# yinyunie/Pose2Room

Measured on AMD Instinct MI355X. Metric: P2RNet train-step samples/sec (T=1024,J=53,bs=32), higher is better.
Workload: dtype f32; 1 GPU; P2RNet full train step, bs=32/GPU, T=1024, J=53, seeds=512, proposals=128 (BASELINE configs[2]); input=P2RNet_dataloader over SyntheticPoseDataset, global_batch=32, frames=1024, parallelism=dp1

## Files before the change

pose2room_amd/p2rnet/modules/stgcn.py:

```python
import torch
import torch.nn as nn

from ..registers import MODULES
from .stgcn_layers import Graph, st_gcn_block
from .sub_modules import SingleConv


def _point_mlp(cin, width, cout):
    return nn.Sequential(SingleConv(cin, width, kernel_size=1, order='cbr', padding=0, ndim=1),
                         SingleConv(width, width, kernel_size=1, order='cbr', padding=0, ndim=1),
                         SingleConv(width, cout, kernel_size=1, order='c', padding=0, ndim=1))


@MODULES.register_module
class STGCN(nn.Module):
    def __init__(self, cfg, optim_spec=None):
        super().__init__()
        self.optim_spec = optim_spec

        self.graph = Graph(layout='virtualroom', strategy='spatial', max_hop=5)
        self.register_buffer('A', torch.tensor(self.graph.A, dtype=torch.float32, requires_grad=False))

        self.n_seeds = cfg.config['data']['num_seeds']
        self.origin_joint_id = cfg.dataset_config.origin_joint_id
        width, out_channels = 64, 256
        kernel_size = (3, self.A.size(0))
        self.knn = 20

        self.pos_embed = _point_mlp(3, 64, width)
        self.sk_feat = _point_mlp(3, 64, width)
        self.st_gcn_networks = nn.ModuleList(
            [st_gcn_block(width, 64, kernel_size, 1, residual=False)] +
            [st_gcn_block(64, 64, kernel_size, 1) for _ in range(5)])
        from ..gcn_op import GraphTables
        tables = GraphTables(self.graph.A)
        for i, blk in enumerate(self.st_gcn_networks):
            blk.gcn.tables = tables
            blk.chain_input = i > 0
        self.conv_joint = nn.Conv1d(cfg.dataset_config.joint_num * 64, out_channels, kernel_size=1)
        self.edge_importance = nn.ParameterList(
            [nn.Parameter(torch.ones(self.A.size())) for _ in self.st_gcn_networks])

        n_frames = cfg.config['data']['num_frames']
        if self.n_seeds >= n_frames:
            self.seed_inds = torch.round(torch.linspace(0, n_frames - 1, self.n_seeds)).long()
        else:
            self.seed_sampling = cfg.config['data']['seed_sampling']

    def _select_seeds(self, hip):
        n_batch, n_frames, _ = hip.shape
        device = hip.device
        if self.n_seeds >= n_frames:
            return self.seed_inds.repeat(n_batch, 1).to(device)
        if self.seed_sampling == 'random':
            inds = torch.argsort(torch.rand(size=(n_batch, n_frames)), dim=1)[:, :self.n_seeds]
            return torch.sort(inds, dim=1)[0].to(device)
        if self.seed_sampling == 'uniform':
            step = torch.norm(torch.diff(hip, dim=1), dim=2)
            cum = torch.cumsum(torch.cat([torch.zeros(size=(n_batch, 1), device=device), step], dim=1).double(),
                               dim=1).float()
            stride = cum[:, -1] / (self.n_seeds - 1)
            target = stride.unsqueeze(-1) * torch.arange(self.n_seeds, dtype=torch.float, device=device)
            if cum.is_cuda and cum.dtype == torch.float32 and n_frames <= 40000:
                from .. import seed_op
                return seed_op.nearest_prefix(cum, target)
            return torch.argmin(torch.abs(cum.unsqueeze(-1) - target.unsqueeze(1)), dim=1)
        raise NotImplementedError

    @staticmethod
    def _mlp(seq, x, inner, add_ct=None):
        from .. import bn_op, tconv_op, embed_op
        if embed_op.supported(seq, x, inner, add_ct):
            return embed_op.embed_mlp(seq, x, inner, add_ct)
        s0, s1, s2 = seq
        fused = (x.is_cuda and len(seq) == 3 and hasattr(s0, 'batchnorm') and hasattr(s1, 'batchnorm')
                 and not hasattr(s2, 'batchnorm') and tconv_op.supported_embed3(x, s0.conv)
                 and x.shape[2] % inner == 0 and inner <= 64)
        if fused:
            z0s = None
            if s0.batchnorm.training:
                z, z0s = tconv_op.embed3(x, s0.conv, want_stats=True)
            else:
                z = tconv_op.embed3(x, s0.conv)
            z = z.view(x.shape[0], 64, x.shape[2] // inner, inner)
            fused = tconv_op.supported_pointwise(z, s0.batchnorm, s1.conv) and \
                tconv_op.supported_pointwise(z, s1.batchnorm, s2.conv)
            if fused:
                if s1.batchnorm.training:
                    z, zs = tconv_op.bn_relu_tconv(z, s0.batchnorm, s1.conv, stats=z0s, want_stats=True)
                    z = tconv_op.bn_relu_tconv(z, s1.batchnorm, s2.conv, stats=zs, add_ct=add_ct)
                else:
                    z = tconv_op.bn_relu_tconv(z, s0.batchnorm, s1.conv)
                    z = tconv_op.bn_relu_tconv(z, s1.batchnorm, s2.conv, add_ct=add_ct)
                return z.view(x.shape[0], 64, x.shape[2])
        for stage in seq:
            if x.is_cuda and hasattr(stage, 'batchnorm') and hasattr(stage, 'ReLU') and \
                    bn_op.supported(x, stage.batchnorm):
                x = bn_op.fused_bn_act(stage.conv(x), stage.batchnorm, None, relu=True)
            else:
                x = stage(x)
        if add_ct is not None:
            x = (x.view(x.shape[0], x.shape[1], -1, inner) + add_ct.unsqueeze(-1)).view(x.shape)
        return x

    def embed(self, input_joints):
        n_batch, n_frames, n_joints, _ = input_joints.shape
        device = input_joints.device
        hip = input_joints[:, :, self.origin_joint_id]
        win = torch.arange(n_frames, device=device).unsqueeze(-1) + \
            torch.arange(-self.knn // 2, self.knn // 2, device=device).unsqueeze(0)
        win = win.clamp_(0, n_frames - 1)
        offs = hip[:, win] - hip.unsqueeze(2)
        pe = self._mlp(self.pos_embed, offs.reshape(n_batch, n_frames * self.knn, 3).transpose(1, 2).contiguous(), self.knn)
        from .. import seed_op
        pe = pe.view(n_batch, -1, n_frames, self.knn)
        fused = seed_op.short_rows_supported(pe)
        pe = seed_op.mean_last(pe) if fused else pe.mean(dim=3)
        rel = input_joints - input_joints[:, :, self.origin_joint_id:self.origin_joint_id + 1]
        sk = self._mlp(self.sk_feat, rel.reshape(n_batch, n_frames * n_joints, 3).transpose(1, 2).contiguous(), n_joints,
                       add_ct=pe)
        return sk.view(n_batch, -1, n_frames, n_joints)

    def forward(self, input_joints, end_points=None):
        end_points = {} if end_points is None else end_points
        n_batch, n_frames, n_joints, n_dim = input_joints.size()
        seed_inds = self._select_seeds(input_joints[:, :, self.origin_joint_id])

        x = self.embed(input_joints)
        blocks = self.st_gcn_networks
        tables = blocks[0].gcn.tables
        if tables is not None and tables.gen2 and all(b.chainable(x, self.A) for b in blocks):
            from ..gcn_op import prepare_chain
            for gcn, prep in zip(blocks, prepare_chain(blocks, self.A, self.edge_importance, tables, frames=x.shape[2])):
                x, _ = gcn(x, prep.Aeff, prepared=prep)
        else:
            for gcn, importance in zip(blocks, self.edge_importance):
                x, _ = gcn(x, self.A * importance)

        seed_skeleton = torch.gather(
            input_joints, 1, seed_inds[:, :, None, None].expand(n_batch, self.n_seeds, n_joints, n_dim))
        if self.n_seeds < n_frames:
            from .. import seed_op
            if seed_op.seed_rows_supported(x, seed_inds):
                rows = seed_op.seed_rows(x, seed_inds)
            else:
                rows = x.permute(0, 2, 1, 3)[torch.arange(n_batch, device=x.device)[:, None], seed_inds]
            seed_features = torch.nn.functional.linear(
                rows.reshape(n_batch, self.n_seeds, -1),
                self.conv_joint.weight.squeeze(-1), self.conv_joint.bias)
        else:
            x = x.transpose(2, 3).reshape(n_batch, -1, n_frames)
            seed_features = self.conv_joint(x).transpose(1, 2)
            seed_features = torch.gather(
                seed_features, 1, seed_inds.unsqueeze(-1).expand(n_batch, self.n_seeds, seed_features.size(-1)))
        end_points['seed_inds'] = seed_inds
        end_points['seed_skeleton'] = seed_skeleton[..., :3]
        end_points['seed_features'] = seed_features
        return end_points
```

pose2room_amd/p2rnet/modules/stgcn_layers.py:

```python
from collections import deque

import numpy as np
import torch
import torch.nn as nn

_VIRTUALROOM_BONES = [
    (0, 1), (1, 3), (3, 5), (5, 19), (0, 2), (2, 4), (4, 6), (6, 20), (0, 7), (7, 8), (8, 9),
    (9, 10), (10, 21), (10, 22), (8, 11), (11, 13), (13, 15), (15, 17), (8, 12), (12, 14),
    (14, 16), (16, 18), (17, 23), (23, 24), (24, 25), (17, 26), (26, 27), (27, 28), (17, 29),
    (29, 30), (30, 31), (17, 32), (32, 33), (33, 34), (17, 35), (35, 36), (36, 37), (18, 38),
    (38, 39), (39, 40), (18, 41), (41, 42), (42, 43), (18, 44), (44, 45), (45, 46), (18, 47),
    (47, 48), (48, 49), (18, 50), (50, 51), (51, 52)]

_LAYOUTS = {'virtualroom': dict(num_node=53, bones=_VIRTUALROOM_BONES, center=0)}


def hop_distance(num_node, edges, max_hop):
    nbr = [[] for _ in range(num_node)]
    for i, j in edges:
        if i != j:
            nbr[i].append(j)
            nbr[j].append(i)
    hop = np.full((num_node, num_node), np.inf)
    for s in range(num_node):
        hop[s, s] = 0
        dq = deque([s])
        while dq:
            u = dq.popleft()
            if hop[s, u] >= max_hop:
                continue
            for v in nbr[u]:
                if np.isinf(hop[s, v]):
                    hop[s, v] = hop[s, u] + 1
                    dq.append(v)
    return hop


class Graph:

    def __init__(self, layout='virtualroom', strategy='spatial', max_hop=5, dilation=1):
        if layout not in _LAYOUTS:
            raise ValueError("Do Not Exist This Layout.")
        spec = _LAYOUTS[layout]
        self.max_hop, self.dilation = max_hop, dilation
        self.num_node, self.center = spec['num_node'], spec['center']
        self.edge = [(i, i) for i in range(self.num_node)] + list(spec['bones'])
        self.hop_dis = hop_distance(self.num_node, self.edge, max_hop)
        self.A = self._adjacency(strategy)

    def _adjacency(self, strategy):
        V = self.num_node
        hops = list(range(0, self.max_hop + 1, self.dilation))
        reach = np.zeros((V, V))
        for h in hops:
            reach[self.hop_dis == h] = 1
        col = reach.sum(0)
        inv = np.zeros(V)
        inv[col > 0] = col[col > 0] ** (-1)
        norm = reach * inv[None, :]
        if strategy == 'uniform':
            return norm[None]
        if strategy == 'distance':
            return np.stack([np.where(self.hop_dis == h, norm, 0.0) for h in hops])
        if strategy == 'spatial':
            dc = self.hop_dis[:, self.center]
            same = dc[:, None] == dc[None, :]
            closer = dc[:, None] > dc[None, :]
            planes = []
            for h in hops:
                at_h = self.hop_dis == h
                root = np.where(at_h & same, norm, 0.0)
                close = np.where(at_h & closer, norm, 0.0)
                further = np.where(at_h & ~same & ~closer, norm, 0.0)
                if h == 0:
                    planes.append(root)
                else:
                    planes.append(root + close)
                    planes.append(further)
            return np.stack(planes)
        raise ValueError("Do Not Exist This Strategy")


class ConvTemporalGraphical(nn.Module):

    def __init__(self, in_channels, out_channels, kernel_size, t_kernel_size=1, t_stride=1,
                 t_padding=0, t_dilation=1, bias=True):
        super().__init__()
        self.kernel_size = kernel_size
        self.out_channels = out_channels
        self.tables = None
        self.fused = True
        self.conv = nn.Conv2d(in_channels, out_channels * kernel_size, kernel_size=(t_kernel_size, 1),
                              padding=(t_padding, 0), stride=(t_stride, 1), dilation=(t_dilation, 1),
                              bias=bias)

    def forward(self, x, A, want_stats=False, with_residual=False, bn_link=None, prepared=None, lazy_res=False):
        assert A.size(0) == self.kernel_size
        if self.tables is not None and self.fused:
            from .. import gcn_op
            if gcn_op.supported(x, self.conv.weight, A):
                return gcn_op.graph_conv(x, self.conv.weight, self.conv.bias, A, self.tables, want_stats,
                                         with_residual, bn_link, prepared, lazy_res), A
        assert not want_stats and not with_residual and prepared is None
        y = self.conv(x)
        n, kc, t, v = y.size()
        y = y.view(n, self.kernel_size, kc // self.kernel_size, t, v)
        z = torch.einsum('nkctv,kvw->nctw', (y, A))
        return z.contiguous(), A


def _zero(x):
    return 0


def _iden(x):
    return x


class st_gcn_block(nn.Module):

    def __init__(self, in_channels, out_channels, kernel_size, stride=1, dropout=0, residual=True):
        super().__init__()
        assert len(kernel_size) == 2 and kernel_size[0] % 2 == 1
        padding = ((kernel_size[0] - 1) // 2, 0)
        self.gcn = ConvTemporalGraphical(in_channels, out_channels, kernel_size[1])
        self.tcn = nn.Sequential(
            nn.BatchNorm2d(out_channels),
            nn.ReLU(inplace=True),
            nn.Conv2d(out_channels, out_channels, (kernel_size[0], 1), (stride, 1), padding),
            nn.BatchNorm2d(out_channels),
            nn.Dropout(dropout, inplace=True),
        )
        if not residual:
            self.residual = _zero
        elif in_channels == out_channels and stride == 1:
            self.residual = _iden
        else:
            self.residual = nn.Sequential(
                nn.Conv2d(in_channels, out_channels, kernel_size=1, stride=(stride, 1)),
                nn.BatchNorm2d(out_channels))
        self.relu = nn.ReLU(inplace=True)

    fused_bn = True
    fused_tconv = True
    lazy_residual_grad = True
    chain_input = False

    def chainable(self, x, A):
        if not (self.fused_bn and x.is_cuda and self.tcn[4].p == 0):
            return False
        from .. import bn_op, gcn_op, tconv_op
        return (self.training and self.fused_tconv and self.gcn.tables is not None and self.gcn.fused
                and gcn_op.supported(x, self.gcn.conv.weight, A) and bn_op.supported(x, self.tcn[0])
                and tconv_op.supported(x, self.tcn[0], self.tcn[2]))

    def forward(self, x, A, prepared=None):
        res = self.residual(x)
        if self.fused_bn and x.is_cuda and self.tcn[4].p == 0:
            from .. import bn_op, gcn_op, tconv_op
            chain = self.chainable(x, A)
            assert chain or prepared is None
            lazy = False
            if chain:
                if self.residual is _iden and x.requires_grad:
                    in_link = getattr(x, '_p2r_bn_link', None) if self.chain_input else None
                    lazy = self.lazy_residual_grad and self.tcn[3].training
                    (z, zstats, res), A = self.gcn(x, A, want_stats=True, with_residual=True, bn_link=in_link,
                                                   prepared=prepared, lazy_res=lazy)
                else:
                    (z, zstats), A = self.gcn(x, A, want_stats=True, prepared=prepared)
                wp = (prepared.tcn_wp_f, prepared.tcn_wp_b) if prepared is not None and z.shape[3] == 53 else None
                u, ustats = tconv_op.bn_relu_tconv(z, self.tcn[0], self.tcn[2], stats=zstats, want_stats=True, wp=wp)
                res_t = res if torch.is_tensor(res) else None
                return bn_op.fused_bn_act(u, self.tcn[3], res_t, relu=True, stats=ustats, link=bn_op.BNLink(),
                                          lazy_res=lazy), A
            x, A = self.gcn(x, A)
            if bn_op.supported(x, self.tcn[0]):
                if self.fused_tconv and tconv_op.supported(x, self.tcn[0], self.tcn[2]):
                    u = tconv_op.bn_relu_tconv(x, self.tcn[0], self.tcn[2])
                else:
                    h = bn_op.fused_bn_act(x, self.tcn[0], None, relu=True)
                    u = self.tcn[2](h)
                res_t = res if torch.is_tensor(res) else None
                return bn_op.fused_bn_act(u, self.tcn[3], res_t, relu=True), A
        else:
            x, A = self.gcn(x, A)
        x = self.tcn(x) + res
        return self.relu(x), A
```

pose2room_amd/p2rnet/seed_op.py:

```python
import torch
from torch.autograd import Function

from .. import _lib


def _rowsum(x, V, scale):
    out = torch.empty(x.shape[:-1], dtype=torch.float32, device=x.device)
    _lib.launch("p2r_rowsum_short", x.device, x.numel() // V, V, scale, x, out)
    return out


def short_rows_supported(x):
    return x.is_cuda and x.dtype == torch.float32 and 1 <= x.shape[-1] <= 64


class _SeedRows(Function):

    @staticmethod
    def forward(ctx, x, seed_inds):
        x = x.contiguous()
        inds = seed_inds.long().contiguous()
        B, C, T, J = x.shape
        S = inds.shape[1]
        out = torch.empty((B, S, C * J), dtype=torch.float32, device=x.device)
        _lib.launch("p2r_gather_frames", x.device, B, C, T, J, S, x, inds, out)
        ctx.save_for_backward(inds)
        ctx.dims = (B, C, T, J, S)
        return out

    @staticmethod
    def backward(ctx, dout):
        (inds,) = ctx.saved_tensors
        B, C, T, J, S = ctx.dims
        dout = dout.contiguous()
        dx = torch.empty((B, C, T, J), dtype=torch.float32, device=dout.device)
        _lib.launch("p2r_gather_frames_grad", dout.device, B, C, T, J, S, dout, inds, dx)
        return dx, None


def seed_rows_supported(x, seed_inds):
    return (x.is_cuda and x.dtype == torch.float32 and x.dim() == 4 and seed_inds.is_cuda and seed_inds.dim() == 2
            and seed_inds.dtype in (torch.int64, torch.int32) and seed_inds.shape[0] == x.shape[0])


def seed_rows(x, seed_inds):
    return _SeedRows.apply(x, seed_inds)


class _MeanLast(Function):

    @staticmethod
    def forward(ctx, x):
        x = x.contiguous()
        ctx.shape = x.shape
        return _rowsum(x, x.shape[-1], 1.0 / x.shape[-1])

    @staticmethod
    def backward(ctx, g):
        return (g * (1.0 / ctx.shape[-1])).unsqueeze(-1).expand(ctx.shape)


def mean_last(x):
    return _MeanLast.apply(x)


class _AddBroadcastLast(Function):

    @staticmethod
    def forward(ctx, a, b):
        ctx.V = a.shape[-1]
        return a + b.unsqueeze(-1)

    @staticmethod
    def backward(ctx, g):
        db = None
        if ctx.needs_input_grad[1]:
            gc = g.contiguous()
            db = _rowsum(gc, ctx.V, 1.0)
        return (g if ctx.needs_input_grad[0] else None), db


def add_broadcast_last(a, b):
    return _AddBroadcastLast.apply(a, b)


def nearest_prefix(cum, target):
    cum, target = cum.contiguous(), target.contiguous()
    B, T = cum.shape
    S = target.shape[1]
    out = torch.empty((B, S), dtype=torch.int64, device=cum.device)
    _lib.launch("p2r_nearest_prefix", cum.device, B, T, S, cum, target, out)
    return out
```

Before: 796.3 samples/s.

## Fuse last ST-GCN block BN+ReLU with seed-frame gather, skip full activation

In training, the final ST-GCN block's output BN+residual+ReLU is now fused with the seed-row gather. It computes activations only at the selected seed frames instead of writing the full B×C×T×J tensor and gathering from it afterwards. The backward pass builds a per-frame linked list of seed indices so duplicate seeds are handled, then runs a BN-statistics reduce kernel and an apply kernel that produce du and dres directly. This saves one full-size write and read in forward, but backward still streams over the full activation and adds an index-building kernel, a uint8 mask, and a second shared library.

```diff
diff --git a/include/p2r_seed_seam.h b/include/p2r_seed_seam.h
--- /dev/null
+++ b/include/p2r_seed_seam.h
@@ -0,0 +1,23 @@
+#ifndef P2R_SEED_SEAM_H
+#define P2R_SEED_SEAM_H
+
+#include "p2r_hip.h"
+
+#ifdef __cplusplus
+extern "C" {
+#endif
+
+int p2r_seam_apply_gather(int b, int c, int t, int j, int s, const float *u, const float *res, const float *scale,
+                          const float *shift, const long long *inds, float *rows, unsigned char *mask, void *stream);
+int p2r_seam_index(int b, int t, int s, const long long *inds, int *head, int *next, void *stream);
+int p2r_seam_bwd_reduce(int b, int c, int t, int j, int s, const float *drows, const unsigned char *mask,
+                        const float *u, const float *mean, const float *invstd, const int *head, const int *next,
+                        float *partial, void *stream);
+int p2r_seam_bwd_apply(int b, int c, int t, int j, int s, const float *drows, const unsigned char *mask,
+                       const float *u, const float *mean, const float *invstd, const float *kscale, const float *m1,
+                       const float *m2, const int *head, const int *next, float *du, float *dres, void *stream);
+
+#ifdef __cplusplus
+}
+#endif
+#endif
diff --git a/pose2room_amd/csrc/seed_seam.hip b/pose2room_amd/csrc/seed_seam.hip
--- /dev/null
+++ b/pose2room_amd/csrc/seed_seam.hip
@@ -0,0 +1,271 @@
+#include "p2r_common.h"
+
+#include "../../include/p2r_seed_seam.h"
+
+namespace {
+
+constexpr int SS_THREADS = 256;
+constexpr int SS_MAX_T = 8192;
+
+typedef float f4v __attribute__((ext_vector_type(4)));
+__device__ __forceinline__ float4 ld_stream(const float *p) {
+  const f4v t = __builtin_nontemporal_load(reinterpret_cast<const f4v *>(p));
+  return make_float4(t.x, t.y, t.z, t.w);
+}
+__device__ __forceinline__ void st_stream(float *p, const float4 &v) {
+  __builtin_nontemporal_store(f4v{v.x, v.y, v.z, v.w}, reinterpret_cast<f4v *>(p));
+}
+
+__global__ __launch_bounds__(SS_THREADS) void seam_index_kernel(int T, int S, const long long *__restrict__ inds,
+                                                               int *__restrict__ head, int *__restrict__ next) {
+  __shared__ long long tile[SS_THREADS];
+  const int b = blockIdx.y, tid = threadIdx.x;
+  const int nT = (T + SS_THREADS - 1) / SS_THREADS;
+  const long long *ib = inds + (size_t)b * S;
+  const bool frames = (int)blockIdx.x < nT;
+  const int id = (frames ? (int)blockIdx.x : (int)blockIdx.x - nT) * SS_THREADS + tid;
+  long long want = -1;
+  int from = 0;
+  if (frames) {
+    if (id < T) want = id;
+  } else if (id < S) {
+    const long long t = ib[id];
+    if (t >= 0 && t < T) want = t;
+    from = id + 1;
+  }
+  int found = -1;
+  for (int s0 = frames ? 0 : ((int)blockIdx.x - nT) * SS_THREADS; s0 < S; s0 += SS_THREADS) {
+    __syncthreads();
+    tile[tid] = s0 + tid < S ? ib[s0 + tid] : -1;
+    __syncthreads();
+    if (want >= 0 && found < 0) {
+      const int n = min(SS_THREADS, S - s0);
+      for (int k = max(0, from - s0); k < n; ++k)
+        if (tile[k] == want) { found = s0 + k; break; }
+    }
+  }
+  if (frames) {
+    if (id < T) head[(size_t)b * T + id] = found;
+  } else if (id < S) {
+    next[(size_t)b * S + id] = found;
+  }
+}
+
+__global__ __launch_bounds__(SS_THREADS) void seam_apply_gather_kernel(int C, int T, int J, int S,
+                                                                      const float *__restrict__ u,
+                                                                      const float *__restrict__ res,
+                                                                      const float *__restrict__ scale,
+                                                                      const float *__restrict__ shift,
+                                                                      const long long *__restrict__ inds,
+                                                                      float *__restrict__ rows,
+                                                                      unsigned char *__restrict__ mask) {
+  const int b = blockIdx.x / S;
+  const long long t = inds[blockIdx.x];
+  const int n = C * J;
+  float *o = rows + (size_t)blockIdx.x * n;
+  unsigned char *m = mask + (size_t)blockIdx.x * n;
+  if (t < 0 || t >= T) {
+    for (int e = threadIdx.x; e < n; e += SS_THREADS) { o[e] = 0.f; m[e] = 0; }
+    return;
+  }
+  const size_t fb = ((size_t)b * C * T + t) * J;
+  for (int e = threadIdx.x; e < n; e += SS_THREADS) {
+    const int c = e / J, j = e - c * J;
+    const size_t at = fb + (size_t)c * T * J + j;
+    float v = fmaf(u[at], scale[c], shift[c]);
+    if (res) v += res[at];
+    v = fmaxf(v, 0.f);
+    o[e] = v;
+    m[e] = v > 0.f;
+  }
+}
+
+__device__ __forceinline__ float seam_gated(const float *__restrict__ rows_c, const unsigned char *__restrict__ mask_c,
+                                            const int *__restrict__ next_b, int S, int h, int n, int j) {
+  const size_t at = (size_t)h * n + j;
+  float g = rows_c[at];
+  const unsigned char m = mask_c[at];
+  for (int nx = next_b[h]; nx >= 0 && nx < S; nx = next_b[nx]) g += rows_c[(size_t)nx * n + j];
+  return m ? g : 0.f;
+}
+
+__device__ __forceinline__ float ss_wave_sum(float v) {
+#pragma unroll
+  for (int off = 32; off >= 1; off >>= 1) v += __shfl_xor(v, off, 64);
+  return v;
+}
+
+__global__ __launch_bounds__(SS_THREADS) void seam_bwd_reduce_kernel(int C, int T, int J, int S,
+                                                                    const float *__restrict__ drows,
+                                                                    const unsigned char *__restrict__ mask,
+                                                                    const float *__restrict__ u,
+                                                                    const float *__restrict__ mean,
+                                                                    const float *__restrict__ invstd,
+                                                                    const int *__restrict__ head,
+                                                                    const int *__restrict__ next,
+                                                                    float2 *__restrict__ partial) {
+  extern __shared__ int s_head[];
+  __shared__ float sa[SS_THREADS / 64], sb[SS_THREADS / 64];
+  const int row = blockIdx.x, b = row / C, c = row - b * C, tid = threadIdx.x;
+  for (int t = tid; t < T; t += SS_THREADS) s_head[t] = head[(size_t)b * T + t];
+  __syncthreads();
+  const float mu = mean[c], is = invstd[c];
+  const int L = T * J, n = C * J;
+  const size_t base = (size_t)row * L;
+  const float *rows_c = drows + (size_t)b * S * n + (size_t)c * J;
+  const unsigned char *mask_c = mask + (size_t)b * S * n + (size_t)c * J;
+  const int *next_b = next + (size_t)b * S;
+  auto term = [&](int e, int t, int j, float &g, float &gx) {
+    const int h = s_head[t];
+    g = 0.f; gx = 0.f;
+    if (h >= 0 && h < S) {
+      g = seam_gated(rows_c, mask_c, next_b, S, h, n, j);
+      gx = g * ((u[base + e] - mu) * is);
+    }
+  };
+  float s = 0.f, q = 0.f;
+  const int L4 = (base % 4 == 0) ? (L >> 2) : 0;
+  for (int i = tid; i < L4; i += SS_THREADS) {
+    const int e = 4 * i;
+    int t = e / J, j = e - t * J;
+    float g[4], gx[4];
+#pragma unroll
+    for (int k = 0; k < 4; ++k) {
+      term(e + k, t, j, g[k], gx[k]);
+      if (++j == J) { j = 0; ++t; }
+    }
+    s += (g[0] + g[1]) + (g[2] + g[3]);
+    q += (gx[0] + gx[1]) + (gx[2] + gx[3]);
+  }
+  for (int e = (L4 << 2) + tid; e < L; e += SS_THREADS) {
+    const int t = e / J;
+    float g, gx;
+    term(e, t, e - t * J, g, gx);
+    s += g; q += gx;
+  }
+  s = ss_wave_sum(s);
+  q = ss_wave_sum(q);
+  if ((tid & 63) == 0) { sa[tid >> 6] = s; sb[tid >> 6] = q; }
+  __syncthreads();
+  if (tid == 0) {
+    s = 0.f; q = 0.f;
+#pragma unroll
+    for (int i = 0; i < SS_THREADS / 64; ++i) { s += sa[i]; q += sb[i]; }
+    partial[row] = make_float2(s, q);
+  }
+}
+
+__global__ __launch_bounds__(SS_THREADS) void seam_bwd_apply_kernel(int C, int T, int J, int S, int chunks,
+                                                                   const float *__restrict__ drows,
+                                                                   const unsigned char *__restrict__ mask,
+                                                                   const float *__restrict__ u,
+                                                                   const float *__restrict__ mean,
+                                                                   const float *__restrict__ invstd,
+                                                                   const float *__restrict__ kscale,
+                                                                   const float *__restrict__ m1,
+                                                                   const float *__restrict__ m2,
+                                                                   const int *__restrict__ head,
+                                                                   const int *__restrict__ next,
+                                                                   float *__restrict__ du, float *__restrict__ dres) {
+  const int rowi = blockIdx.x / chunks, chunk = blockIdx.x % chunks;
+  const int b = rowi / C, c = rowi - b * C;
+  const float mu = mean[c], is = invstd[c], kk = kscale[c], a1 = m1[c], a2 = m2[c];
+  const int L = T * J, n = C * J;
+  const size_t base = (size_t)rowi * L;
+  const int per = (((L + chunks - 1) / chunks) + 3) & ~3;
+  const int lo = chunk * per, hi = min(L, lo + per);
+  const float *rows_c = drows + (size_t)b * S * n + (size_t)c * J;
+  const unsigned char *mask_c = mask + (size_t)b * S * n + (size_t)c * J;
+  const int *next_b = next + (size_t)b * S, *head_b = head + (size_t)b * T;
+  auto one = [&](int t, int j, float xv, float &dxo, float &dro) {
+    const int h = head_b[t];
+    const float g = (h >= 0 && h < S) ? seam_gated(rows_c, mask_c, next_b, S, h, n, j) : 0.f;
+    const float xh = (xv - mu) * is;
+    dxo = kk * (g - a1 - xh * a2);
+    dro = g;
+  };
+  const bool vec = (((uintptr_t)(u + base) | (uintptr_t)(du + base) | (dres ? (uintptr_t)(dres + base) : 0)) % 16 == 0);
+  int tail = lo;
+  if (vec) {
+    tail = lo + ((hi - lo) & ~3);
+    for (int e = lo + threadIdx.x * 4; e + 3 < hi; e += SS_THREADS * 4) {
+      const float4 x4 = ld_stream(u + base + e);
+      const float xs[4] = {x4.x, x4.y, x4.z, x4.w};
+      float o[4], r[4];
+      int t = e / J, j = e - t * J;
+#pragma unroll
+      for (int k = 0; k < 4; ++k) {
+        one(t, j, xs[k], o[k], r[k]);
+        if (++j == J) { j = 0; ++t; }
+      }
+      st_stream(du + base + e, make_float4(o[0], o[1], o[2], o[3]));
+      if (dres) st_stream(dres + base + e, make_float4(r[0], r[1], r[2], r[3]));
+    }
+  }
+  for (int e = tail + threadIdx.x; e < hi; e += SS_THREADS) {
+    const int t = e / J;
+    float o, r;
+    one(t, e - t * J, u[base + e], o, r);
+    du[base + e] = o;
+    if (dres) dres[base + e] = r;
+  }
+}
+
+static int seam_chunks(int rows, int L) {
+  int chunks = 1;
+  while ((long long)rows * chunks < 2048 && (L / (chunks * 2)) >= 4096) chunks *= 2;
+  return chunks;
+}
+
+static bool seam_dims_ok(int b, int c, int t, int j, int s) {
+  return b >= 0 && c > 0 && t > 0 && j > 0 && s > 0 && (long long)t * j <= 0x7fffffffLL && (long long)c * j <= 0x7fffffffLL &&
+         (long long)b * c <= 0x7fffffffLL && (long long)b * s <= 0x7fffffffLL;
+}
+
+}
+
+extern "C" int p2r_seam_index(int b, int t, int s, const long long *inds, int *head, int *next, void *stream) {
+  if (b < 0 || t <= 0 || s <= 0 || b > 65535) return P2R_EINVAL;
+  if (b == 0) return P2R_OK;
+  const unsigned nx = (unsigned)((t + SS_THREADS - 1) / SS_THREADS + (s + SS_THREADS - 1) / SS_THREADS);
+  hipLaunchKernelGGL(seam_index_kernel, dim3(nx, (unsigned)b), dim3(SS_THREADS), 0, p2r_stream(stream), t, s, inds, head, next);
+  P2R_LAUNCH_CHECK();
+  return P2R_OK;
+}
+
+extern "C" int p2r_seam_apply_gather(int b, int c, int t, int j, int s, const float *u, const float *res, const float *scale,
+                                     const float *shift, const long long *inds, float *rows, unsigned char *mask,
+                                     void *stream) {
+  if (!seam_dims_ok(b, c, t, j, s)) return P2R_EINVAL;
+  if (b == 0) return P2R_OK;
+  hipLaunchKernelGGL(seam_apply_gather_kernel, dim3((unsigned)(b * s)), dim3(SS_THREADS), 0, p2r_stream(stream), c, t, j, s, u,
+                     res, scale, shift, inds, rows, mask);
+  P2R_LAUNCH_CHECK();
+  return P2R_OK;
+}
+
+extern "C" int p2r_seam_bwd_reduce(int b, int c, int t, int j, int s, const float *drows, const unsigned char *mask,
+                                   const float *u, const float *mean, const float *invstd, const int *head, const int *next,
+                                   float *partial, void *stream) {
+  if (!seam_dims_ok(b, c, t, j, s) || t > SS_MAX_T) return P2R_EINVAL;
+  if (b == 0) return P2R_OK;
+  hipLaunchKernelGGL(seam_bwd_reduce_kernel, dim3((unsigned)(b * c)), dim3(SS_THREADS), (size_t)t * sizeof(int),
+                     p2r_stream(stream), c, t, j, s, drows, mask, u, mean, invstd, head, next,
+                     reinterpret_cast<float2 *>(partial));
+  P2R_LAUNCH_CHECK();
+  return P2R_OK;
+}
+
+extern "C" int p2r_seam_bwd_apply(int b, int c, int t, int j, int s, const float *drows, const unsigned char *mask,
+                                  const float *u, const float *mean, const float *invstd, const float *kscale,
+                                  const float *m1, const float *m2, const int *head, const int *next, float *du, float *dres,
+                                  void *stream) {
+  if (!seam_dims_ok(b, c, t, j, s)) return P2R_EINVAL;
+  if (b == 0) return P2R_OK;
+  const int rows = b * c, chunks = seam_chunks(rows, t * j);
+  if ((long long)rows * chunks > 0x7fffffffLL) return P2R_EINVAL;
+  hipLaunchKernelGGL(seam_bwd_apply_kernel, dim3((unsigned)(rows * chunks)), dim3(SS_THREADS), 0, p2r_stream(stream), c, t, j, s,
+                     chunks, drows, mask, u, mean, invstd, kscale, m1, m2, head, next, du, dres);
+  P2R_LAUNCH_CHECK();
+  return P2R_OK;
+}
diff --git a/pose2room_amd/p2rnet/modules/stgcn.py b/pose2room_amd/p2rnet/modules/stgcn.py
--- a/pose2room_amd/p2rnet/modules/stgcn.py
+++ b/pose2room_amd/p2rnet/modules/stgcn.py
@@ -129,10 +129,14 @@
         x = self.embed(input_joints)
         blocks = self.st_gcn_networks
         tables = blocks[0].gcn.tables
+        rows = None
         if tables is not None and tables.gen2 and all(b.chainable(x, self.A) for b in blocks):
             from ..gcn_op import prepare_chain
+            seam = self.n_seeds < n_frames and blocks[-1].seam_supported(x, self.A, seed_inds)
             for gcn, prep in zip(blocks, prepare_chain(blocks, self.A, self.edge_importance, tables, frames=x.shape[2])):
-                x, _ = gcn(x, prep.Aeff, prepared=prep)
+                x, _ = gcn(x, prep.Aeff, prepared=prep, seed_inds=seed_inds if seam and gcn is blocks[-1] else None)
+            if seam:
+                rows, x = x, None
         else:
             for gcn, importance in zip(blocks, self.edge_importance):
                 x, _ = gcn(x, self.A * importance)
@@ -141,7 +145,9 @@
             input_joints, 1, seed_inds[:, :, None, None].expand(n_batch, self.n_seeds, n_joints, n_dim))
         if self.n_seeds < n_frames:
             from .. import seed_op
-            if seed_op.seed_rows_supported(x, seed_inds):
+            if rows is not None:
+                pass
+            elif seed_op.seed_rows_supported(x, seed_inds):
                 rows = seed_op.seed_rows(x, seed_inds)
             else:
                 rows = x.permute(0, 2, 1, 3)[torch.arange(n_batch, device=x.device)[:, None], seed_inds]
diff --git a/pose2room_amd/p2rnet/modules/stgcn_layers.py b/pose2room_amd/p2rnet/modules/stgcn_layers.py
--- a/pose2room_amd/p2rnet/modules/stgcn_layers.py
+++ b/pose2room_amd/p2rnet/modules/stgcn_layers.py
@@ -154,17 +154,25 @@
                 and gcn_op.supported(x, self.gcn.conv.weight, A) and bn_op.supported(x, self.tcn[0])
                 and tconv_op.supported(x, self.tcn[0], self.tcn[2]))
 
-    def forward(self, x, A, prepared=None):
+    def seam_supported(self, x, A, seed_inds):
+        if not (self.fused_bn and x.is_cuda and self.tcn[4].p == 0 and self.residual is _iden):
+            return False
+        from .. import seed_op
+        from torch.nn.modules import module as _m
+        hooked = bool(self._forward_hooks) or bool(_m._global_forward_hooks)
+        return not hooked and self.chainable(x, A) and seed_op.seam_supported(x, self.tcn[3], seed_inds)
+
+    def forward(self, x, A, prepared=None, seed_inds=None):
         res = self.residual(x)
         if self.fused_bn and x.is_cuda and self.tcn[4].p == 0:
-            from .. import bn_op, gcn_op, tconv_op
+            from .. import bn_op, gcn_op, seed_op, tconv_op
             chain = self.chainable(x, A)
-            assert chain or prepared is None
+            assert chain or (prepared is None and seed_inds is None)
             lazy = False
             if chain:
                 if self.residual is _iden and x.requires_grad:
                     in_link = getattr(x, '_p2r_bn_link', None) if self.chain_input else None
-                    lazy = self.lazy_residual_grad and self.tcn[3].training
+                    lazy = self.lazy_residual_grad and self.tcn[3].training and seed_inds is None
                     (z, zstats, res), A = self.gcn(x, A, want_stats=True, with_residual=True, bn_link=in_link,
                                                    prepared=prepared, lazy_res=lazy)
                 else:
@@ -172,6 +180,8 @@
                 wp = (prepared.tcn_wp_f, prepared.tcn_wp_b) if prepared is not None and z.shape[3] == 53 else None
                 u, ustats = tconv_op.bn_relu_tconv(z, self.tcn[0], self.tcn[2], stats=zstats, want_stats=True, wp=wp)
                 res_t = res if torch.is_tensor(res) else None
+                if seed_inds is not None:
+                    return seed_op.bn_act_seed_rows(u, self.tcn[3], res_t, seed_inds, stats=ustats), A
                 return bn_op.fused_bn_act(u, self.tcn[3], res_t, relu=True, stats=ustats, link=bn_op.BNLink(),
                                           lazy_res=lazy), A
             x, A = self.gcn(x, A)
diff --git a/pose2room_amd/p2rnet/seed_op.py b/pose2room_amd/p2rnet/seed_op.py
--- a/pose2room_amd/p2rnet/seed_op.py
+++ b/pose2room_amd/p2rnet/seed_op.py
@@ -1,3 +1,6 @@
+import ctypes
+import os
+
 import torch
 from torch.autograd import Function
 
@@ -47,6 +50,97 @@
     return _SeedRows.apply(x, seed_inds)
 
 
+SEAM_HEADER_PATH = os.path.join(os.path.dirname(_lib.HEADER_PATH), "p2r_seed_seam.h")
+SEAM_LIB_PATH = os.path.join(os.path.dirname(os.path.abspath(_lib.__file__)), "libp2r_seed_seam.so")
+_seam_lib = None
+_seam_protos = None
+
+
+def seam_lib():
+    global _seam_lib, _seam_protos
+    if _seam_lib is None:
+        if not os.path.exists(SEAM_LIB_PATH):
+            raise _lib.P2RLibraryError(f"{SEAM_LIB_PATH} is missing: build it with `make -C pose2room_amd/csrc` "
+                                       "(pose2room_amd has no CPU fallback)")
+        l = ctypes.CDLL(SEAM_LIB_PATH)
+        _seam_protos = _lib.prototypes(SEAM_HEADER_PATH)
+        for name, proto in _seam_protos.items():
+            fn = getattr(l, name)
+            fn.restype, fn.argtypes = proto.restype, proto.argtypes
+        _seam_lib = l
+    return _seam_lib
+
+
+def seam_launch(name, device, *args):
+    l = seam_lib()
+    proto = _seam_protos[name]
+    if len(args) != len(proto.pointer):
+        raise TypeError(f"{name}: {len(args)} arguments for {len(proto.pointer)} parameters in front of the stream: {proto.text}")
+    vals = [(a.data_ptr() if a is not None else None) if p else int(a) for a, p in zip(args, proto.pointer)]
+    if device.index is None or device.index == torch.cuda.current_device():
+        _lib.check(getattr(l, name)(*vals, _lib.current_stream(device)), name)
+    else:
+        with torch.cuda.device(device):
+            _lib.check(getattr(l, name)(*vals, _lib.current_stream(device)), name)
+
+
+FUSE_SEAM = True
+SEAM_MAX_FRAMES = 8192
+
+
+class _SeamBNAct(Function):
+
+    @staticmethod
+    def forward(ctx, u, weight, bias, res, fin, seed_inds):
+        u = u.contiguous()
+        res_c = res.contiguous() if res is not None else None
+        inds = seed_inds.long().contiguous()
+        B, C, T, J = u.shape
+        S = inds.shape[1]
+        rows = torch.empty((B, S, C * J), dtype=torch.float32, device=u.device)
+        mask = torch.empty((B, S, C * J), dtype=torch.uint8, device=u.device)
+        seam_launch("p2r_seam_apply_gather", u.device, B, C, T, J, S, u, res_c, fin[2], fin[3], inds, rows, mask)
+        ctx.save_for_backward(u, mask, fin, inds)
+        ctx.dims = (B, C, T, J, S)
+        ctx.has_res = res is not None
+        return rows
+
+    @staticmethod
+    def backward(ctx, drows):
+        from . import bn_op
+        u, mask, fin, inds = ctx.saved_tensors
+        B, C, T, J, S = ctx.dims
+        dev = u.device
+        drows = drows.contiguous()
+        head = torch.empty((B, T), dtype=torch.int32, device=dev)
+        nxt = torch.empty((B, S), dtype=torch.int32, device=dev)
+        seam_launch("p2r_seam_index", dev, B, T, S, inds, head, nxt)
+        part = torch.empty((B, C, 2), dtype=torch.float32, device=dev)
+        seam_launch("p2r_seam_bwd_reduce", dev, B, C, T, J, S, drows, mask, u, fin[0], fin[1], head, nxt, part)
+        tot = bn_op.bwd_finalize(part, B * T * J)
+        du = torch.empty_like(u)
+        dres = torch.empty_like(u) if (ctx.has_res and ctx.needs_input_grad[3]) else None
+        seam_launch("p2r_seam_bwd_apply", dev, B, C, T, J, S, drows, mask, u, fin[0], fin[1], fin[2], tot[2], tot[3], head, nxt,
+                    du, dres)
+        return du, tot[1], tot[0], dres, None, None
+
+
+def seam_supported(x, bn, seed_inds):
+    from . import bn_op, math_mode
+    return (FUSE_SEAM and bn.training and not math_mode.split16() and x.dim() == 4 and bn_op.supported(x, bn)
+            and seed_inds is not None and seed_rows_supported(x, seed_inds)
+            and 0 < seed_inds.shape[1] < x.shape[2] <= SEAM_MAX_FRAMES and 0 < x.shape[0] <= 65535)
+
+
+def bn_act_seed_rows(u, bn, res, seed_inds, stats=None):
+    from . import bn_op
+    part = bn_op._stats_partial(u.contiguous()) if stats is None else stats
+    fin = bn_op.finalize(part, u.numel() // u.shape[1], bn)
+    if bn_op.GATE_HOOK is not None:
+        bn_op.GATE_HOOK(bn, u, fin[2], fin[3], res)
+    return _SeamBNAct.apply(u, bn.weight, bn.bias, res, fin, seed_inds)
+
+
 class _MeanLast(Function):
 
     @staticmethod
```

New measurement: 794.9 samples/s. No clear change (-0.2%).
